# MGI-tech-bioinformatics/SuperPlus

Hardware: AMD Instinct MI355X
Metric: k-mers/s (DF createDict stage: trim + canonical k-mer count + solid filter + spectrum + adjacency) (higher is better)
Workload: dtype u64

## Files before the change

superplus_amd/csrc/dfk.hip:

```cpp
#include "../../include/dfk.h"
#include "dfk_kernels.h"
#include "dfk_arena.h"
#include "dfk_adj_plan.h"

#include <algorithm>
#include <chrono>
#include <cstdarg>
#include <cstdio>
#include <cstdlib>
#include <cstring>
#include <atomic>
#include <fcntl.h>
#include <functional>
#include <new>
#include <string>
#include <sys/mman.h>
#include <sys/stat.h>
#include <unistd.h>
#include <condition_variable>
#include <memory>
#include <mutex>
#include <numeric>
#include <thread>
#include <vector>
// ... 214 lines not shown
int device_scan(dfk_ctx* c, const uint64_t* in, uint64_t* out, uint64_t n)
{
    constexpr uint64_t PER = (uint64_t)SCAN_THREADS * SCAN_ITEMS;
    if (n == 0) return 0;
    const uint64_t nblk = (n + PER - 1) / PER;
    if (nblk == 1) {
        hipLaunchKernelGGL(k_scan_blocks, dim3(1), dim3(SCAN_THREADS), 0, c->stream, in, out, n, (uint64_t*)nullptr);
        HIP_TRY(hipGetLastError());
        return 0;
    }
    DevBuf sums; int rc = c->alloc(sums, nblk * 8, "scan block sums"); if (rc) return rc;
    hipLaunchKernelGGL(k_scan_blocks, dim3((unsigned)nblk), dim3(SCAN_THREADS), 0, c->stream, in, out, n, (uint64_t*)sums.p);
    HIP_TRY(hipGetLastError());
    rc = device_scan(c, (const uint64_t*)sums.p, (uint64_t*)sums.p, nblk); if (rc) return rc;
    hipLaunchKernelGGL(k_scan_add, dim3((unsigned)nblk), dim3(SCAN_THREADS), 0, c->stream, out, n, (const uint64_t*)sums.p);
    HIP_TRY(hipGetLastError());
    HIP_TRY(hipStreamSynchronize(c->stream));
    c->release(sums);
    return 0;
}

struct BucketTable {
    uint32_t log2_nb = 0;
    DevBuf acc;
    DevBuf summ;
    DevBuf classes;
    DevBuf ovf_list; uint64_t n_ovf = 0;
    DevBuf class_hist;
    std::vector<uint64_t> h_class;
    uint64_t n_records = 0, n_inst = 0;
};
struct Partition {
    DevBuf records, base, ipre, items;
    uint64_t n_records = 0, n_inst = 0, n_items = 0;
    uint64_t nb = 0;
};

template <int K>
PartParams part_params(const dfk_ctx* c, uint32_t log2_nb, uint32_t log2_world, int64_t read_id0, uint32_t sub_lo, uint32_t sub_n)
{
    const uint32_t M = c->cfg.minimizer_len;
    return PartParams{M, (uint32_t)K - M + 1, log2_nb, log2_world, read_id0, sub_lo, sub_n,
                      sweep_class_mask(sub_lo, sub_n, log2_nb - log2_world)};
}

int table_totals(dfk_ctx* c, const DevBuf& acc, uint64_t nb, uint64_t* n_records, uint64_t* n_inst)
{
    DevBuf tot; int rc = c->alloc(tot, 16, "bucket totals"); if (rc) return rc;
    HIP_TRY(hipMemsetAsync(tot.p, 0, 16, c->stream));
    hipLaunchKernelGGL(k_sum_acc, dim3(1024), dim3(256), 0, c->stream, (const unsigned long long*)acc.p, nb, (unsigned long long*)tot.p);
    HIP_TRY(hipGetLastError());
    uint64_t h[2];
    HIP_TRY(hipMemcpyAsync(h, tot.p, 16, hipMemcpyDeviceToHost, c->stream));
    HIP_TRY(hipStreamSynchronize(c->stream));
    c->release(tot);
    *n_records = h[0]; *n_inst = h[1];
    return 0;
}

struct ScanJob {
    PartParams pp; ScanPlan plan;
    DevBuf ovf_tmp, d_n;
    DevBuf keys, keys2, fill, sub;
    uint64_t n_pieces = 0; bool count_due = false;
    hipEvent_t ev_scan = nullptr, ev_count = nullptr, ev_part[2] = {nullptr, nullptr};
    std::vector<std::pair<hipEvent_t, hipEvent_t>> ev;
    ~ScanJob()
    {
        for (auto& e : ev) { (void)hipEventDestroy(e.first); (void)hipEventDestroy(e.second); }
        for (hipEvent_t e : {ev_scan, ev_count, ev_part[0], ev_part[1]}) if (e) (void)hipEventDestroy(e);
    }
};

template <int K> bool scan_takes_ranges(const dfk_ctx* c) { return c->cfg.minimizer_len == 16; }

ScanSwitches scan_switches()
{
    static const uint32_t scan_blocks = getenv("DFK_SCAN_BLOCKS") ? (uint32_t)atoi(getenv("DFK_SCAN_BLOCKS")) : 0;
    ScanSwitches sw;
    sw.scan_blocks = scan_blocks;
    if (const char* e = getenv("DFK_SCAN_KEY_PIECE")) { sw.key_piece_set = true; sw.key_piece = strtoull(e, nullptr, 10); }
    if (const char* e = getenv("DFK_SCAN_KEY_TAIL")) sw.key_tail = strtoull(e, nullptr, 10);
    sw.no_overlap = getenv("DFK_NO_OVERLAP") != nullptr;
    return sw;
}

template <int K>
int scan_begin(dfk_ctx* c, const Inputs& in, uint32_t log2_world, int64_t read_id0, BucketTable* T, bool by_class, ScanJob* J)
{
    J->pp = part_params<K>(c, T->log2_nb, log2_world, read_id0, 0, 1u << (T->log2_nb - log2_world));
    J->plan = plan_scan(ScanInputs{K, J->pp.W, T->log2_nb, log2_world, in.n_reads, in.packed_bytes, by_class, scan_takes_ranges<K>(c), c->stream2 != nullptr, scan_switches()});
    ScanPlan& P = J->plan;
    int rc = 0;
    if (by_class) { rc = c->alloc(T->class_hist, P.n_bins * 8, "class counters", Place::Low); if (rc) return rc; HIP_TRY(hipMemsetAsync(T->class_hist.p, 0, P.n_bins * 8, c->stream)); }
    else { rc = c->alloc(T->acc, P.nb * 8, "bucket counters", Place::Low); if (rc) return rc; }
    rc = c->alloc(T->summ, std::max<uint64_t>(1, in.n_reads) * 16, "run summaries", Place::Low); if (rc) return rc;
    rc = c->alloc(T->classes, std::max<uint64_t>(1, in.n_reads) * 4, "read bucket classes", Place::Low); if (rc) return rc;
    if (!by_class) HIP_TRY(hipMemsetAsync(T->acc.p, 0, P.nb * 8, c->stream));
    rc = c->alloc(J->ovf_tmp, P.ovf_cap * 4, "overflow read list (scratch)"); if (rc) return rc;
    rc = c->alloc(J->d_n, 16, "overflow read count"); if (rc) return rc;
    HIP_TRY(hipMemsetAsync(J->d_n.p, 0, 16, c->stream));
    if (P.keyed) {
        size_scan_keys(P, c->largest_allocatable());
        rc = c->alloc(J->keys, P.keys_bytes, "run keys (scratch)"); if (rc) return rc;
        rc = c->alloc(J->keys2, P.keys2_bytes, "run keys by sub-slice (scratch)"); if (rc) return rc;
        rc = c->alloc(J->fill, P.fill_bytes, "run key slice fills (scratch)"); if (rc) return rc;
        rc = c->alloc(J->sub, P.sub_bytes, "run key sub-slices (scratch)"); if (rc) return rc;
        if (P.n_slices > 1)
            for (hipEvent_t* e : {&J->ev_scan, &J->ev_count, &J->ev_part[0], &J->ev_part[1]}) HIP_TRY(hipEventCreateWithFlags(e, hipEventDisableTiming));
        TRACE("run keys: %u x %u classes of %llu keys, %u sub-slices each, pieces of %llu reads", P.n_slices, P.n_cls, (unsigned long long)P.cap,
              P.n_sub, (unsigned long long)P.piece_reads);
    }
    return 0;
}

inline int scan_keys_count(dfk_ctx* c, BucketTable* T, ScanJob* J)
{
    const ScanPlan& P = J->plan;
    const uint64_t n_subs = P.n_subs();
    const auto* off = (const unsigned long long*)J->sub.p + n_subs;
    if (P.n_slices > 1) HIP_TRY(hipStreamWaitEvent(c->stream, J->ev_part[scan_piece_step(P, J->n_pieces - 1).slice], 0));
    hipLaunchKernelGGL(k_keys_count, dim3((unsigned)n_subs), dim3(1024), 0, c->stream,
                       (const uint32_t*)J->keys2.p, off, P.sb, (unsigned long long*)T->acc.p);
    HIP_TRY(hipGetLastError());
    if (P.n_slices > 1) HIP_TRY(hipEventRecord(J->ev_count, c->stream));
    J->count_due = false;
    return 0;
}

template <int K>
int scan_keys_piece(dfk_ctx* c, const Inputs& in, BucketTable* T, ScanJob* J, uint64_t r0, uint64_t r1)
{
    const ScanPlan& P = J->plan;
    const unsigned cus = (unsigned)c->prop.multiProcessorCount;
    const unsigned grid = scan_grid(P, r1 - r0, cus);
    const uint64_t n_subs = P.n_subs();
    const bool two = P.n_slices > 1;
    const PieceStep step = scan_piece_step(P, J->n_pieces);
    const uint32_t sl = step.slice;
    hipStream_t ks = two ? c->stream2 : c->stream;
    auto* cnt = (unsigned long long*)J->sub.p;
    auto* off = cnt + n_subs;
    auto* cur = off + n_subs + 1;
    ScanKeys sk{(uint32_t*)J->keys.p + (uint64_t)sl * P.cap * P.n_cls, (unsigned long long*)J->fill.p + (uint64_t)sl * P.n_cls, P.cap, P.ib};
    if (step.wait_slice_reader) HIP_TRY(hipStreamWaitEvent(c->stream, J->ev_part[sl], 0));
    HIP_TRY(hipMemsetAsync(sk.fill, 0, P.n_cls * 8, c->stream));
    hipLaunchKernelGGL(HIP_KERNEL_NAME(k_scan_count<K, 16, true>), dim3(grid), dim3(PART_THREADS), scan_lds(P), c->stream,
                       in.packed, in.packed_bytes, in.base_off, (const uint32_t*)c->good_len.p, r0, r1, J->pp,
                       (unsigned long long*)T->acc.p, (unsigned long long*)nullptr, (unsigned long long*)J->d_n.p, P.ovf_cap,
                       (uint32_t*)J->ovf_tmp.p, (uint4*)T->summ.p, (uint32_t*)T->classes.p, sk);
    HIP_TRY(hipGetLastError());
    if (two) {
        HIP_TRY(hipEventRecord(J->ev_scan, c->stream));
        if (J->count_due) { int rc = scan_keys_count(c, T, J); if (rc) return rc; }
        HIP_TRY(hipStreamWaitEvent(ks, J->ev_scan, 0));
        if (step.wait_prev_count) HIP_TRY(hipStreamWaitEvent(ks, J->ev_count, 0));
    }
    HIP_TRY(hipMemsetAsync(cnt, 0, n_subs * 8, ks));
    const dim3 per_class(std::max(1u, 16u * cus / P.n_cls), P.n_cls);
    const uint32_t sh = 6 + P.sb;
    hipLaunchKernelGGL(k_keys_subcount, per_class, dim3(256), P.n_sub * 4, ks,
                       (const uint32_t*)sk.keys, (const unsigned long long*)sk.fill, sk.cap, sh, P.n_sub, cnt);
    HIP_TRY(hipGetLastError());
    hipLaunchKernelGGL(k_keys_offsets, dim3(1), dim3(1024), 0, ks, (const unsigned long long*)cnt, (uint32_t)n_subs, off, cur);
    HIP_TRY(hipGetLastError());
    hipLaunchKernelGGL(k_keys_partition, per_class, dim3(256), P.n_sub * 12, ks,
                       (const uint32_t*)sk.keys, (const unsigned long long*)sk.fill, sk.cap, sh, P.n_sub, cur, (uint32_t*)J->keys2.p);
    HIP_TRY(hipGetLastError());
    if (two) HIP_TRY(hipEventRecord(J->ev_part[sl], ks));
    ++J->n_pieces; J->count_due = true;
    if (!two) return scan_keys_count(c, T, J);
    return 0;
}

template <int K>
int scan_range(dfk_ctx* c, const Inputs& in, BucketTable* T, ScanJob* J, uint64_t r0, uint64_t r1)
{
    if (r1 <= r0) return 0;
    const PartParams& pp = J->pp;
    const ScanPlan& P = J->plan;
    const unsigned grid = scan_grid(P, r1 - r0, (unsigned)c->prop.multiProcessorCount);
    hipEvent_t e0, e1;
    HIP_TRY(hipEventCreate(&e0)); HIP_TRY(hipEventCreate(&e1));
    J->ev.emplace_back(e0, e1);
    HIP_TRY(hipEventRecord(e0, c->stream));
    if (P.keyed) {
        uint64_t p0 = r0;
        for (uint64_t m : scan_piece_sizes(P, r1 - r0, r1 == in.n_reads)) {
            int rc = scan_keys_piece<K>(c, in, T, J, p0, p0 + m); if (rc) return rc;
            p0 += m;
        }
        if (r1 == in.n_reads && J->count_due) { int rc = scan_keys_count(c, T, J); if (rc) return rc; }
    } else if (P.register_scan) {
        hipLaunchKernelGGL(HIP_KERNEL_NAME(k_scan_count<K, 16, false>), dim3(grid), dim3(PART_THREADS), scan_lds(P), c->stream,
                           in.packed, in.packed_bytes, in.base_off, (const uint32_t*)c->good_len.p, r0, r1, pp,
                           (unsigned long long*)T->acc.p, (unsigned long long*)T->class_hist.p, (unsigned long long*)J->d_n.p, P.ovf_cap,
                           (uint32_t*)J->ovf_tmp.p, (uint4*)T->summ.p, (uint32_t*)T->classes.p, ScanKeys{});
    } else {
        if (r0 != 0 || r1 != in.n_reads) return fail(DFK_E_STATE, "the general scan takes every read at once");
        hipLaunchKernelGGL(HIP_KERNEL_NAME(k_partition<K, false>), dim3(grid), dim3(PART_THREADS), scan_lds(P), c->stream,
                           in.packed, in.packed_bytes, in.base_off, (const uint32_t*)c->good_len.p, in.bc,
                           (int64_t)c->cfg.ign_bc_below, in.n_reads, pp, (unsigned long long*)T->acc.p, (unsigned long long*)T->class_hist.p,
                           (unsigned long long*)J->d_n.p, P.ovf_cap, (uint4*)J->ovf_tmp.p, (uint4*)T->summ.p,
                           (const uint32_t*)nullptr, (uint64_t)0, (const uint64_t*)nullptr, (uint32_t*)T->classes.p);
    }
    HIP_TRY(hipGetLastError());
    HIP_TRY(hipEventRecord(e1, c->stream));
    return 0;
}

template <int K>
int scan_end(dfk_ctx* c, const Inputs& in, uint64_t n_inst, BucketTable* T, ScanJob* J)
{
    int rc = 0;
    T->n_ovf = 0;
    if (J->count_due) { rc = scan_keys_count(c, T, J); if (rc) return rc; }
    c->release(J->keys); c->release(J->keys2); c->release(J->fill); c->release(J->sub);
    if (in.n_reads) {
        HIP_TRY(hipMemcpyAsync(&T->n_ovf, J->d_n.p, 8, hipMemcpyDeviceToHost, c->stream));
        HIP_TRY(hipStreamSynchronize(c->stream));
        if (T->n_ovf > J->plan.ovf_cap) {
            c->release(J->ovf_tmp);
            rc = c->alloc(J->ovf_tmp, in.n_reads * 4, "overflow read list (scratch)"); if (rc) return rc;
            HIP_TRY(hipMemsetAsync(J->d_n.p, 0, 16, c->stream));
            hipLaunchKernelGGL(k_select_overflow, dim3((unsigned)std::min<uint64_t>((in.n_reads + 255) / 256, 8192)), dim3(256), 0, c->stream,
                               (const uint4*)T->summ.p, in.n_reads, (uint32_t*)J->ovf_tmp.p, (unsigned long long*)J->d_n.p);
            HIP_TRY(hipGetLastError());
            HIP_TRY(hipMemcpyAsync(&T->n_ovf, J->d_n.p, 8, hipMemcpyDeviceToHost, c->stream));
            HIP_TRY(hipStreamSynchronize(c->stream));
        }
        if (T->n_ovf) {
            rc = c->alloc(T->ovf_list, T->n_ovf * 4, "overflow read list", Place::Low); if (rc) return rc;
            HIP_TRY(hipMemcpyAsync(T->ovf_list.p, J->ovf_tmp.p, T->n_ovf * 4, hipMemcpyDeviceToDevice, c->stream));
            HIP_TRY(hipStreamSynchronize(c->stream));
        }
    }
    c->release(J->ovf_tmp); c->release(J->d_n);
    HIP_TRY(hipStreamSynchronize(c->stream));
    float ms = 0;
    for (auto& e : J->ev) { float m = 0; if (hipEventElapsedTime(&m, e.first, e.second) == hipSuccess) ms += m; }
    c->st.ms_part_count = ms; c->st.reserved[6] = J->ev.size();
    TRACE("%llu of %llu reads have more than %d runs", (unsigned long long)T->n_ovf, (unsigned long long)in.n_reads, SUMMARY_RUNS);
    const uint64_t nb = J->plan.nb, n_bins = J->plan.n_bins;
    if (J->plan.by_class) {
        T->h_class.assign(n_bins, 0);
        HIP_TRY(hipMemcpyAsync(T->h_class.data(), T->class_hist.p, n_bins * 8, hipMemcpyDeviceToHost, c->stream));
        HIP_TRY(hipStreamSynchronize(c->stream));
        T->n_records = T->n_inst = 0;
        for (uint64_t i = 0; i < n_bins / 2; ++i) { T->n_records += T->h_class[i]; T->n_inst += T->h_class[n_bins / 2 + i]; }
    } else { rc = table_totals(c, T->acc, nb, &T->n_records, &T->n_inst); if (rc) return rc; }
    TRACE("partition count pass done (%llu buckets, %llu records%s)", (unsigned long long)nb, (unsigned long long)T->n_records, J->ev.size() > 1 ? ", in ranges under the upload" : "");
    if (T->n_inst != n_inst)
        return fail(DFK_E_HIP, "partition count pass saw %llu instances, trim saw %llu%s",
                    (unsigned long long)T->n_inst, (unsigned long long)n_inst,
                    (n_inst - T->n_inst) % (1ull << 32) == 0 ? " (a fine bucket with 2^32 or more instances: its counter keeps 32 bits)" : "");
    c->st.n_records = T->n_records; c->st.n_buckets = nb;
    return 0;
}

template <int K>
int partition_count(dfk_ctx* c, const Inputs& in, uint64_t n_inst, uint32_t log2_world, int64_t read_id0, BucketTable* T, bool by_class = false)
{
    ScanJob J;
    int rc = scan_begin<K>(c, in, log2_world, read_id0, T, by_class, &J); if (rc) return rc;
    rc = scan_range<K>(c, in, T, &J, 0, in.n_reads); if (rc) return rc;
    return scan_end<K>(c, in, n_inst, T, &J);
}

int pass_tables(dfk_ctx* c, const DevBuf& acc, uint32_t log2_sub, uint32_t world, uint32_t sub_lo, uint32_t sub_n, uint64_t budget, Partition* P)
{
    P->nb = (uint64_t)world * sub_n;
    const uint64_t nb = P->nb;
    DevBuf rec, inst, flags, idx;
    int rc = c->alloc(rec, (nb + 1) * 8, "bucket record counts"); if (rc) return rc;
    rc = c->alloc(inst, (nb + 1) * 8, "bucket instance counts"); if (rc) return rc;
    rc = c->alloc(P->base, (nb + 1) * 8, "bucket bases"); if (rc) return rc;
    rc = c->alloc(P->ipre, (nb + 1) * 8, "bucket instance prefix"); if (rc) return rc;
// ... 1564 lines not shown
```

superplus_amd/csrc/dfk_kernels.h:

```cpp
#pragma once
#include <type_traits>
#include "dfk_device.h"
#include "dfk_fallback.h"
#include "dfk_scan_plan.h"

namespace dfk {

template <int K>
__global__ void __launch_bounds__(256)
k_trim(const uint8_t* __restrict__ pq, const uint64_t* __restrict__ pq_off, uint64_t pq_nbytes,
       const uint64_t* __restrict__ base_off, uint64_t packed_bytes, const uint32_t* __restrict__ read_len,
       uint64_t n_reads, uint32_t min_qual, uint32_t* __restrict__ good_len,
       unsigned long long* __restrict__ n_inst, unsigned int* __restrict__ bad,
       unsigned long long* __restrict__ sum_good)
{
    unsigned long long mine = 0, good = 0;
    bool any_bad = false;
    for (uint64_t r = (uint64_t)blockIdx.x * blockDim.x + threadIdx.x; r < n_reads; r += (uint64_t)gridDim.x * blockDim.x) {
        uint32_t gl = 0;
        uint64_t p = pq_off[r], end = pq_off[r + 1];
        uint32_t idx = 0, run = 0;
        const uint64_t b0 = base_off[r], b1 = base_off[r + 1];
        bool ok = p <= end && end <= pq_nbytes && b0 <= b1 && b1 <= packed_bytes && b1 - b0 >= ((uint64_t)read_len[r] + 3) / 4;
        if (!ok) end = p;
// ... 11 lines not shown
                idx += nQs;
            } else {
                uint64_t bit = 8 * (p + 1) + 9;
                const uint32_t fmask = (1u << nBits) - 1u;
                for (uint32_t left = nQs; left;) {
                    const uint64_t by = bit >> 3;
                    const uint32_t sh = (uint32_t)(bit & 7);
                    uint64_t w = 0;
                    if (by + 8 <= pq_nbytes) __builtin_memcpy(&w, pq + by, 8);
                    else for (uint32_t k = 0; k < 8 && by + k < pq_nbytes; ++k) w |= (uint64_t)pq[by + k] << (8 * k);
                    w >>= sh;
                    const uint32_t n = min(left, (64u - sh) / nBits);
                    for (uint32_t i = 0; i < n; ++i, w >>= nBits) {
                        const uint32_t q = minQ + ((uint32_t)w & fmask);
                        if (q < min_qual) run = 0;
                        else if (++run >= (uint32_t)K) gl = idx + 1;
                        ++idx;
                    }
                    bit += (uint64_t)n * nBits; left -= n;
                }
            }
            p += blk;
        }
        uint32_t rl = read_len[r];
        if (!ok || idx != rl) { any_bad = true; gl = 0; }
        if (gl > rl) gl = rl;
        good_len[r] = gl;
        good += gl;
        if (gl >= (uint32_t)K + 1) mine += gl - K + 1;
    }
    __shared__ unsigned long long sh[2][4];
    __shared__ unsigned int sh_bad;
    if (threadIdx.x == 0) sh_bad = 0;
    __syncthreads();
#pragma unroll
    for (int d = 32; d > 0; d >>= 1) { mine += __shfl_down(mine, d, 64); good += __shfl_down(good, d, 64); }
    if ((threadIdx.x & 63) == 0) { sh[0][threadIdx.x >> 6] = mine; sh[1][threadIdx.x >> 6] = good; }
    if (any_bad) atomicOr(&sh_bad, 1u);
    __syncthreads();
    if (threadIdx.x == 0) {
        unsigned long long a0 = sh[0][0] + sh[0][1] + sh[0][2] + sh[0][3], a1 = sh[1][0] + sh[1][1] + sh[1][2] + sh[1][3];
        if (a0) atomicAdd(n_inst, a0);
        if (a1) atomicAdd(sum_good, a1);
        if (sh_bad) atomicOr(bad, 1u);
    }
}

struct PartParams {
    uint32_t M;
    uint32_t W;
    uint32_t log2_nb;
    uint32_t log2_world;
    int64_t  read_id0;
    uint32_t sub_lo;
    uint32_t sub_n;
    uint32_t class_mask;
};

constexpr uint32_t SWEEP_CLASSES = 32;
__host__ __device__ inline uint32_t sweep_class_of(uint32_t local_bucket, uint32_t log2_local)
{ return log2_local > 5 ? local_bucket >> (log2_local - 5) : local_bucket; }
__host__ __device__ inline uint32_t sweep_class_mask(uint32_t sub_lo, uint32_t sub_n, uint32_t log2_local)
{
    if (sub_n == 0) return 0u;
    const uint32_t a = sweep_class_of(sub_lo, log2_local), b = sweep_class_of(sub_lo + sub_n - 1, log2_local);
    const uint32_t upto_b = b >= 31 ? 0xFFFFFFFFu : ((1u << (b + 1)) - 1u);
    return upto_b & ~((1u << a) - 1u);
}

constexpr uint32_t SUMMARY_OVERFLOW = 15;

__device__ __forceinline__ uint32_t pass_local(uint32_t bucket, const PartParams& pp)
{
    const uint32_t ls = pp.log2_nb - pp.log2_world;
    const uint32_t d = (bucket & ((1u << ls) - 1u)) - pp.sub_lo;
    return d < pp.sub_n ? (bucket >> ls) * pp.sub_n + d : 0xFFFFFFFFu;
}

__device__ __forceinline__ uint32_t bucket_of(uint32_t minhash, const PartParams& pp)
{
    const uint32_t b = (minhash * 0x9E3779B1u) >> (32 - pp.log2_nb);
    return ((b & ((1u << pp.log2_world) - 1u)) << (pp.log2_nb - pp.log2_world)) | (b >> pp.log2_world);
}
constexpr int PART_QCAP = 8;

template <int K>
__device__ __forceinline__ void emit_record(const uint32_t* __restrict__ words, uint64_t n_words, uint64_t bit0,
                                            uint32_t s0, uint32_t nk, uint32_t bucket, uint32_t gl, int32_t tag,
                                            uint64_t dst_index, uint4* __restrict__ records)
{
    const bool hp = s0 > 0;
    const bool hs = s0 + nk + (uint32_t)K <= gl;
    uint64_t bo = bit0 + 2ull * (hp ? s0 - 1 : 0);
    uint64_t wi = bo >> 5; uint32_t sh = (uint32_t)bo & 31u;
    uint32_t w[7];
#pragma unroll
    for (int i = 0; i < 7; ++i) w[i] = (wi + i < n_words) ? words[wi + i] : 0u;
    uint32_t o[6];
#pragma unroll
    for (int i = 0; i < 6; ++i) o[i] = alignbit(w[i + 1], w[i], sh);
    if (!hp) {
#pragma unroll
        for (int i = 5; i > 0; --i) o[i] = (o[i] << 2) | (o[i - 1] >> 30);
        o[0] <<= 2;
    }
    uint32_t nbits = 2u * (1u + nk + (uint32_t)K - 1u + (hs ? 1u : 0u));
#pragma unroll
    for (int i = 0; i < 6; ++i) {
        uint32_t lo = 32u * i;
        if (nbits <= lo) o[i] = 0;
        else if (nbits < lo + 32u) o[i] &= (1u << (nbits - lo)) - 1u;
    }
    uint4 a{rec_header(nk, hp, hs, bucket), (uint32_t)tag, o[0], o[1]};
    uint4 b{o[2], o[3], o[4], o[5]};
    records[2 * dst_index] = a;
    records[2 * dst_index + 1] = b;
}

__device__ __forceinline__ uint32_t class_bin(uint32_t bucket, const PartParams& pp)
{
    const uint32_t ls = pp.log2_nb - pp.log2_world;
    const uint32_t sub = bucket & ((1u << ls) - 1u);
    return (bucket >> ls) * PART_CLASSES + (ls > 6 ? sub >> (ls - 6) : sub);
}

template <int K, bool WRITE>
__device__ __forceinline__ void
partition_read(uint64_t r, uint32_t* smem, uint32_t* __restrict__ lh,
            const uint8_t* __restrict__ packed, uint64_t packed_bytes, const uint64_t* __restrict__ base_off,
            const uint32_t* __restrict__ good_len, const int32_t* __restrict__ bc, int64_t ign_bc_below,
            uint64_t n_reads, const PartParams& pp,
            unsigned long long* __restrict__ bucket_acc, unsigned long long* __restrict__ bucket_cur, uint64_t n_out,
            uint4* __restrict__ records, uint4* __restrict__ summaries, const uint32_t* __restrict__ read_list, uint64_t n_list,
            const uint64_t* __restrict__ slice_base, uint32_t* __restrict__ read_classes)
{
    auto place = [&](uint32_t b) -> uint64_t {
        if (!slice_base) { const uint64_t d = atomicAdd(&bucket_cur[b], 1ull); return d < n_out ? d : ~0ull; }
        const uint32_t owner = b / pp.sub_n;
        const uint64_t d = slice_base[owner] + atomicAdd(&bucket_cur[owner], 1ull);
        return d < slice_base[owner + 1] ? d : ~0ull;
    };
    uint32_t* arr = smem;
    uint32_t* queue = smem + pp.W * PART_THREADS;
    uint8_t* sidx = reinterpret_cast<uint8_t*>(smem + pp.W * PART_THREADS);
    uint32_t* ring = reinterpret_cast<uint32_t*>(sidx + pp.W * PART_THREADS);
    uint64_t sum_lo = 0, sum_hi = 0;
    const int tid = threadIdx.x;
    if (WRITE && read_list) { if (r >= n_list) return; r = read_list[r]; }
    const uint32_t M = pp.M, W = pp.W;
    const uint32_t gl = r < n_reads ? good_len[r] : 0;
    if (gl < (uint32_t)K + 1) {
        if (!WRITE && r < n_reads) { summaries[r] = uint4{0, 0, 0, 0}; if (read_classes) read_classes[r] = 0u; }
        return;
    }
    uint32_t Pi = 0, cur_rel = 0;
    uint32_t cmask = 0;
    const uint32_t log2_local = pp.log2_nb - pp.log2_world;

    const uint64_t byte0 = base_off[r];
    const uint32_t* words = reinterpret_cast<const uint32_t*>(packed);
    const uint64_t n_words = (packed_bytes + 3) >> 2;
    const uint64_t bit0 = byte0 * 8;
    int32_t tag = -1;
    if (bc && (int64_t)r + pp.read_id0 >= ign_bc_below) tag = bc[r];

    const uint32_t mmask = M == 16 ? 0xFFFFFFFFu : ((1u << (2 * M)) - 1u);
// ... 82 lines not shown
        if (++bi == W) {
            uint32_t run = h, ri = W - 1;
            if (!WRITE) sidx[(W - 1) * PART_THREADS + tid] = (uint8_t)(W - 1);
            for (int i0 = (int)W - 2; i0 >= 0; i0 -= 8) {
                uint32_t v[8];
#pragma unroll
                for (int k = 0; k < 8; ++k) v[k] = i0 - k >= 0 ? arr[(i0 - k) * PART_THREADS + tid] : 0u;
#pragma unroll
                for (int k = 0; k < 8; ++k) {
                    const int i = i0 - k;
                    if (i >= 0) {
                        const bool lt = v[k] < run;
                        run = lt ? v[k] : run;
                        arr[i * PART_THREADS + tid] = run;
                        if (!WRITE) { ri = lt ? (uint32_t)i : ri; sidx[i * PART_THREADS + tid] = (uint8_t)ri; }
                    }
                }
            }
            bi = 0;
        }
        if (bi + 1 < W) sfx_next = arr[(bi + 1) * PART_THREADS + tid];
    }
    close_run();
    if (!WRITE) {
        const uint64_t lo = sum_lo | (qn <= (uint32_t)SUMMARY_RUNS ? qn : SUMMARY_OVERFLOW), hi = sum_hi;
        summaries[r] = uint4{(uint32_t)lo, (uint32_t)(lo >> 32), (uint32_t)hi, (uint32_t)(hi >> 32)};
        if (read_classes) read_classes[r] = cmask;
        if (qn > (uint32_t)SUMMARY_RUNS && bucket_cur) {
            const unsigned long long at = atomicAdd(bucket_cur, 1ull);
            if (at < n_out) reinterpret_cast<uint32_t*>(records)[at] = (uint32_t)r;
        }
    }
    if (WRITE) {
        for (uint32_t e = 0; e < qn; ++e) {
            uint32_t a = queue[(2 * e) * PART_THREADS + tid], b = queue[(2 * e + 1) * PART_THREADS + tid];
            const uint64_t dst = place(b);
            if (dst != ~0ull) emit_record<K>(words, n_words, bit0, a & 0xFFFFu, a >> 16, b, gl, tag, dst, records);
        }
    }
}

template <int K, bool WRITE>
__global__ void __launch_bounds__(PART_THREADS)
k_partition(const uint8_t* __restrict__ packed, uint64_t packed_bytes, const uint64_t* __restrict__ base_off,
            const uint32_t* __restrict__ good_len, const int32_t* __restrict__ bc, int64_t ign_bc_below,
            uint64_t n_reads, PartParams pp,
            unsigned long long* __restrict__ bucket_acc,
            unsigned long long* __restrict__ class_hist,
            unsigned long long* __restrict__ bucket_cur,
            uint64_t n_out,
            uint4* __restrict__ records,
            uint4* __restrict__ summaries,
            const uint32_t* __restrict__ read_list,
            uint64_t n_list,
            const uint64_t* __restrict__ slice_base,
            uint32_t* __restrict__ read_classes)
{
    extern __shared__ uint32_t smem[];
    uint32_t* lh = nullptr;
    const uint32_t n_bins = 2u * (PART_CLASSES << pp.log2_world);
    if (!WRITE && class_hist) {
        lh = reinterpret_cast<uint32_t*>(reinterpret_cast<uint8_t*>(smem) + 5 * pp.W * PART_THREADS + 4 * PART_RING * PART_THREADS);
        for (uint32_t i = threadIdx.x; i < n_bins; i += PART_THREADS) lh[i] = 0;
        __syncthreads();
    }
    const uint64_t n_work = (WRITE && read_list) ? n_list : n_reads;
    for (uint64_t r0 = (uint64_t)blockIdx.x * PART_THREADS; r0 < n_work; r0 += (uint64_t)gridDim.x * PART_THREADS)
        partition_read<K, WRITE>(r0 + threadIdx.x, smem, lh, packed, packed_bytes, base_off, good_len, bc, ign_bc_below, n_reads, pp,
                                 bucket_acc, bucket_cur, n_out, records, summaries, read_list, n_list, slice_base, read_classes);
    if (lh) {
        __syncthreads();
        for (uint32_t i = threadIdx.x; i < n_bins; i += PART_THREADS) if (lh[i]) atomicAdd(&class_hist[i], (unsigned long long)lh[i]);
    }
}

template <int I, int N, class F>
__device__ __forceinline__ void static_for(F&& f)
{
    if constexpr (I < N) { f(std::integral_constant<int, I>{}); static_for<I + 1, N>(f); }
}

constexpr uint32_t KEY_TILE = 4096;

template <int K, int M, bool KEYS>
__global__ void __launch_bounds__(PART_THREADS)
k_scan_count(const uint8_t* __restrict__ packed, uint64_t packed_bytes, const uint64_t* __restrict__ base_off,
             const uint32_t* __restrict__ good_len, uint64_t r_first, uint64_t n_reads , PartParams pp,
             unsigned long long* __restrict__ bucket_acc, unsigned long long* __restrict__ class_hist,
             unsigned long long* __restrict__ ovf_count, uint64_t ovf_cap, uint32_t* __restrict__ ovf_list,
             uint4* __restrict__ summaries, uint32_t* __restrict__ read_classes, ScanKeys sk)
{
    constexpr int W = K - M + 1;
    constexpr uint32_t mmask = M == 16 ? 0xFFFFFFFFu : ((1u << (2 * M)) - 1u);
    constexpr uint32_t rsh = 2 * (M - 1);
    constexpr int RUNS = SUMMARY_RUNS;
    static_assert(KTraits<K>::NK_MAX < 64, "nk takes the key's six low bits");
    extern __shared__ uint32_t smem[];
    uint32_t* runb = smem;
    uint16_t* runf = reinterpret_cast<uint16_t*>(runb + RUNS * PART_THREADS);
    uint32_t* const after_runs = reinterpret_cast<uint32_t*>(runf + RUNS * PART_THREADS);
    uint32_t* lh = nullptr;
    const uint32_t n_bins = 2u * (PART_CLASSES << pp.log2_world);
    if (class_hist) {
        lh = after_runs;
        for (uint32_t i = threadIdx.x; i < n_bins; i += PART_THREADS) lh[i] = 0;
        __syncthreads();
    }
    const int tid = threadIdx.x;
    uint32_t* st_key = after_runs;
    unsigned long long* st_base = reinterpret_cast<unsigned long long*>(st_key + SCAN_STAGE);
    uint32_t* st_h = reinterpret_cast<uint32_t*>(st_base + PART_CLASSES);
    uint32_t* st_n = st_h + PART_CLASSES;
    uint8_t* st_cls = reinterpret_cast<uint8_t*>(st_n + 1);
    const uint32_t n_cls = 1u << (pp.log2_nb - sk.ib);
    if constexpr (KEYS) {
        if (tid < PART_CLASSES) st_h[tid] = 0;
        if (tid == 0) *st_n = 0;
        __syncthreads();
    }
    auto flush = [&]() {
        const uint32_t n = *st_n;
        if (tid < (int)n_cls) { const uint32_t h = st_h[tid]; if (h) st_base[tid] = atomicAdd(&sk.fill[tid], (unsigned long long)h); st_h[tid] = 0; }
        __syncthreads();
        for (uint32_t j = tid; j < n; j += PART_THREADS) {
            const uint32_t key = st_key[j], cls = st_cls[j];
            const unsigned long long at = st_base[cls] + atomicAdd(&st_h[cls], 1u);
            if (at < sk.cap) sk.keys[cls * sk.cap + at] = key;
            else atomicAdd(&bucket_acc[(cls << sk.ib) | (key >> 6)], (1ull << 32) | (key & 63u));
        }
        __syncthreads();
        if (tid < (int)n_cls) st_h[tid] = 0;
        if (tid == 0) *st_n = 0;
        __syncthreads();
    };
    const uint32_t* words = reinterpret_cast<const uint32_t*>(packed);
    const uint64_t n_words = (packed_bytes + 3) >> 2;
    const uint32_t log2_local = pp.log2_nb - pp.log2_world;
    for (uint64_t r0 = r_first + (uint64_t)blockIdx.x * PART_THREADS; r0 < n_reads; r0 += (uint64_t)gridDim.x * PART_THREADS) {
        const uint64_t r = r0 + tid;
        const uint32_t gl = r < n_reads ? good_len[r] : 0;
        const bool live = gl >= (uint32_t)K + 1;
        uint32_t qn = 0, cmask = 0;
        uint64_t sum_lo = 0, sum_hi = 0;
        if (live) {
            const uint64_t bit0 = base_off[r] * 8;
            constexpr int NW = (2 * W + 30 + 31) / 32, NA = (2 * W + 31) / 32;
            auto load = [&](uint64_t bit, uint32_t (&w)[NW]) {
                const uint64_t wi = bit >> 5;
#pragma unroll
                for (int k = 0; k < NW; ++k) {
                    const uint64_t i = wi + k;
                    const uint32_t v = words[i < n_words ? i : n_words - 1];
                    w[k] = i < n_words ? v : 0u;
                }
            };
            uint64_t nbit = bit0 + 2 * (M - 1);
            uint32_t nw[NW];
            load(nbit, nw);
            uint32_t f = 0, rc = 0;
            {
                const uint64_t wi = bit0 >> 5;
                const uint32_t w0 = words[wi < n_words ? wi : n_words - 1], w1 = words[wi + 1 < n_words ? wi + 1 : n_words - 1];
                const uint32_t pw = alignbit(wi + 1 < n_words ? w1 : 0u, wi < n_words ? w0 : 0u, (uint32_t)bit0 & 31u);
#pragma unroll
                for (int j = 0; j < M - 1; ++j) { const uint32_t b = (pw >> (2 * j)) & 3u; f = ((f << 2) | b) & mmask; rc = (rc >> 2) | ((3u - b) << rsh); }
            }
            const uint32_t n_mmers = gl - M + 1;
            uint32_t arr[W], sidxw[(W + 3) / 4];
            auto sidx_get = [&](int i) -> uint32_t { return (sidxw[i >> 2] >> (8 * (i & 3))) & 255u; };
            auto sidx_set = [&](int i, uint32_t v) { const uint32_t sh = 8u * (uint32_t)(i & 3); sidxw[i >> 2] = (sidxw[i >> 2] & ~(255u << sh)) | (v << sh); };
#pragma unroll
            for (int i = 0; i < (W + 3) / 4; ++i) sidxw[i] = 0;
            uint32_t P = 0, Pi = 0;
            uint32_t cur_b = 0, cur_nk = 0, cur_rel = 0;
            auto close_run = [&]() {
                if (qn < (uint32_t)RUNS) {
                    runb[qn * PART_THREADS + tid] = cur_b;
                    runf[qn * PART_THREADS + tid] = (uint16_t)(cur_nk | (cur_rel << 6));
                } else {
                    if (lh) { const uint32_t bin = class_bin(cur_b, pp); atomicAdd(&lh[bin], 1u); atomicAdd(&lh[(PART_CLASSES << pp.log2_world) + bin], cur_nk); }
                    else atomicAdd(&bucket_acc[cur_b], (1ull << 32) | cur_nk);
                    cmask |= 1u << sweep_class_of(cur_b & ((1u << log2_local) - 1u), log2_local);
                }
                ++qn;
            };
            for (uint32_t t0 = 0; t0 < n_mmers; t0 += W) {
                uint32_t a[NA];
                {
                    const uint32_t sh = (uint32_t)nbit & 31u;
#pragma unroll
                    for (int i = 0; i < NA; ++i) a[i] = alignbit(i + 1 < NW ? nw[i + 1] : 0u, nw[i], sh);
                }
                nbit += 2 * W;
                load(nbit, nw);
                static_for<0, W>([&](auto bi_c) {
                    constexpr int bi = decltype(bi_c)::value;
                    if (t0 + (uint32_t)bi < n_mmers) {
                        const uint32_t b = (a[(2 * bi) >> 5] >> ((2 * bi) & 31)) & 3u;
                        f = ((f << 2) | b) & mmask;
                        rc = (rc >> 2) | ((3u - b) << rsh);
                        const uint32_t h = mmer_hash(f < rc ? f : rc);
                        const bool newmin = bi == 0 || h < P;
                        P = newmin ? h : P;
                        Pi = newmin ? (uint32_t)bi : Pi;
                        const bool first = t0 == 0;
                        if (!first || bi == W - 1) {
                            uint32_t mv = P;
                            bool older = false;
                            if constexpr (bi != W - 1) { older = arr[bi + 1] < mv; mv = older ? arr[bi + 1] : mv; }
                            const uint32_t bucket = bucket_of(mv, pp);
                            const bool open = first || bucket != cur_b || cur_nk == (uint32_t)KTraits<K>::NK_MAX;
                            if (open && !first) close_run();
                            const uint32_t rel = (bi != W - 1 && older) ? sidx_get(bi + 1 < W ? bi + 1 : 0) - (uint32_t)bi - 1u : (uint32_t)(W - 1 - bi) + Pi;
                            cur_rel = open ? rel : cur_rel;
                            cur_nk = open ? 1u : cur_nk + 1u;
                            cur_b = open ? bucket : cur_b;
                        }
                        arr[bi] = h;
                        if (bi == W - 1) {
                            uint32_t run = h, ri = W - 1;
                            sidx_set(W - 1, W - 1);
                            static_for<0, W - 1>([&](auto j_c) {
                                constexpr int i = W - 2 - decltype(j_c)::value;
                                const bool lt = arr[i] < run; run = lt ? arr[i] : run; arr[i] = run; ri = lt ? (uint32_t)i : ri; sidx_set(i, ri);
                            });
                        }
                    }
                });
            }
            close_run();
        }
        const uint32_t mine = min(qn, (uint32_t)RUNS);
        for (uint32_t i = 0; KEYS ? __syncthreads_or(i < mine) != 0 : __ballot(i < mine) != 0ull; ++i) {
            const bool has = i < mine;
            uint32_t cb = 0, nk = 0;
            if (has) {
                cb = runb[i * PART_THREADS + tid];
                const uint64_t fld = runf[i * PART_THREADS + tid];
                nk = (uint32_t)fld & 63u;
                const uint32_t bfld = 8u + 12u * i;
                if (bfld < 64u) { sum_lo |= fld << bfld; if (bfld > 52u) sum_hi |= fld >> (64u - bfld); } else sum_hi |= fld << (bfld - 64u);
                if constexpr (!KEYS) {
                    if (lh) { const uint32_t bin = class_bin(cb, pp); atomicAdd(&lh[bin], 1u); atomicAdd(&lh[(PART_CLASSES << pp.log2_world) + bin], nk); }
                    else atomicAdd(&bucket_acc[cb], (1ull << 32) | nk);
                }
                cmask |= 1u << sweep_class_of(cb & ((1u << log2_local) - 1u), log2_local);
            }
            if constexpr (KEYS) {
                const uint64_t m = __ballot(has);
                if (m) {
                    const uint32_t rk = __builtin_amdgcn_mbcnt_hi((uint32_t)(m >> 32), __builtin_amdgcn_mbcnt_lo((uint32_t)m, 0u));
                    const int lead = __ffsll((unsigned long long)m) - 1;
                    uint32_t at = 0;
                    if (has && rk == 0) at = atomicAdd(st_n, (uint32_t)__popcll(m));
                    at = __shfl(at, lead) + rk;
                    if (has) {
                        const uint32_t cls = cb >> sk.ib;
                        st_key[at] = ((cb & ((1u << sk.ib) - 1u)) << 6) | nk;
                        st_cls[at] = (uint8_t)cls;
                        atomicAdd(&st_h[cls], 1u);
                    }
                }
                __syncthreads();
                if (*st_n > (uint32_t)(SCAN_STAGE - PART_THREADS)) flush();
            }
        }
        if (r < n_reads) {
            const uint64_t lo = sum_lo | (qn <= (uint32_t)SUMMARY_RUNS ? qn : SUMMARY_OVERFLOW);
            summaries[r] = uint4{(uint32_t)lo, (uint32_t)(lo >> 32), (uint32_t)sum_hi, (uint32_t)(sum_hi >> 32)};
            if (read_classes) read_classes[r] = cmask;
        }
        if (qn > (uint32_t)SUMMARY_RUNS) {
            const unsigned long long at = atomicAdd(ovf_count, 1ull);
            if (at < ovf_cap) ovf_list[at] = (uint32_t)r;
        }
    }
    if constexpr (KEYS) { __syncthreads(); if (*st_n) flush(); }
    if (lh) {
        __syncthreads();
        for (uint32_t i = threadIdx.x; i < n_bins; i += PART_THREADS) if (lh[i]) atomicAdd(&class_hist[i], (unsigned long long)lh[i]);
    }
}

constexpr int KEY_VECS = 4;
static_assert(KEY_TILE == 256u * 4u * KEY_VECS, "a tile is KEY_VECS 16-byte vectors per thread of a 256-thread block");
__device__ __forceinline__ uint32_t key_vec_n(uint64_t t0, uint64_t t1, int j)
{
    const uint64_t i = t0 + ((uint64_t)j * 256u + threadIdx.x) * 4u;
    return i < t1 ? (uint32_t)min((uint64_t)4, t1 - i) : 0u;
}
__device__ __forceinline__ void key_tile_load(const uint32_t* __restrict__ k, uint64_t t0, uint64_t t1, uint4 (&v)[KEY_VECS])
{
#pragma unroll
    for (int j = 0; j < KEY_VECS; ++j) {
        const uint64_t i = t0 + ((uint64_t)j * 256u + threadIdx.x) * 4u;
        v[j] = i < t1 ? *reinterpret_cast<const uint4*>(k + i) : make_uint4(0u, 0u, 0u, 0u);
    }
}
template <typename F>
__device__ __forceinline__ void key_tile_each(uint64_t t0, uint64_t t1, const uint4 (&v)[KEY_VECS], F&& f)
{
#pragma unroll
    for (int j = 0; j < KEY_VECS; ++j) {
        const uint32_t m = key_vec_n(t0, t1, j);
        if (m > 0) f(v[j].x);
        if (m > 1) f(v[j].y);
        if (m > 2) f(v[j].z);
        if (m > 3) f(v[j].w);
        __builtin_amdgcn_sched_barrier(0);
    }
}

__global__ void __launch_bounds__(256)
k_keys_subcount(const uint32_t* __restrict__ keys, const unsigned long long* __restrict__ fill, uint64_t cap, uint32_t sh ,
// ... 1704 lines not shown
```

superplus_amd/csrc/dfk_scan_plan.h:

```cpp
#pragma once
#include <algorithm>
#include <cstddef>
#include <cstdint>
#include <vector>
#include "dfk_fallback.h"

namespace dfk {

constexpr int PART_THREADS = 128;
constexpr int PART_RING = 2;
constexpr int SUMMARY_RUNS = 10;
constexpr uint32_t PART_CLASSES = 64;

struct ScanKeys {
    uint32_t* keys;
    unsigned long long* fill;
    uint64_t cap;
    uint32_t ib;
};
constexpr int SCAN_STAGE = 1536;
constexpr uint32_t KEY_SUB_BITS = 14;
constexpr size_t SCAN_RUN_LDS = (sizeof(uint32_t) + sizeof(uint16_t)) * SUMMARY_RUNS * PART_THREADS;
constexpr size_t SCAN_STAGE_LDS = (sizeof(uint32_t) + 1) * SCAN_STAGE + (sizeof(unsigned long long) + sizeof(uint32_t)) * PART_CLASSES + sizeof(uint32_t);
static_assert(SCAN_RUN_LDS + SCAN_STAGE_LDS <= 16384, "ten scan blocks a CU (160 KB of LDS)");

constexpr uint64_t SCAN_TAIL_READS = 32ull << 20;
constexpr uint64_t KEY_SCRATCH_MAX = 16ull << 30;
constexpr uint32_t SCAN_BLOCKS_PER_CU = 128;

struct ScanSwitches {
    bool key_piece_set = false; uint64_t key_piece = 0;
    uint64_t key_tail = SCAN_TAIL_READS;
    uint32_t scan_blocks = 0;
    bool no_overlap = false;
};

struct ScanInputs {
    int K; uint32_t W, log2_nb, log2_world;
    uint64_t n_reads, packed_bytes;
    bool by_class;
    bool register_scan;
    bool second_stream;
    ScanSwitches sw;
};

struct ScanPlan {
    ScanSwitches sw;
    uint32_t W = 0; uint64_t nb = 0, n_bins = 0, ovf_cap = 0; bool by_class = false, register_scan = false;
    bool keyed = false; uint32_t n_cls = 0, ib = 0, sb = 0, n_sub = 0, n_slices = 1;
    double keys_per_read = 0.0;
    uint64_t n_reads = 0, cap = 0, piece_reads = 0, tail_reads = 0;
    uint64_t keys_bytes = 0, keys2_bytes = 0, fill_bytes = 0, sub_bytes = 0;
    uint64_t n_subs() const { return (uint64_t)n_cls * n_sub; }
};

inline uint64_t ovf_cap(uint64_t n_reads) { return n_reads / 16 + 1024; }

inline ScanPlan plan_scan(const ScanInputs& in)
{
    ScanPlan p;
    p.sw = in.sw; p.W = in.W; p.n_reads = in.n_reads; p.by_class = in.by_class; p.register_scan = in.register_scan;
    p.nb = 1ull << in.log2_nb;
    p.n_bins = 2ull * (PART_CLASSES << in.log2_world);
    p.ovf_cap = ovf_cap(in.n_reads);
    const double runs = in.n_reads ? 1.0 + 2.0 * std::max(0.0, 4.0 * (double)in.packed_bytes / (double)in.n_reads - in.K + 1) / (in.W + 1) : 0.0;
    p.keyed = !in.by_class && in.register_scan && in.n_reads && (runs >= 3.5 || in.sw.key_piece_set);
    if (!p.keyed) return p;
    const uint32_t cb = std::min<uint32_t>(6, in.log2_nb);
    p.ib = in.log2_nb - cb; p.n_cls = 1u << cb;
    p.sb = std::min(KEY_SUB_BITS, p.ib); p.n_sub = 1u << (p.ib - p.sb);
    p.keys_per_read = 1.25 * runs;
    p.n_slices = in.second_stream && !in.sw.no_overlap ? 2 : 1;
    p.tail_reads = in.sw.key_tail;
    return p;
}

inline void size_scan_keys(ScanPlan& p, uint64_t largest_allocatable)
{
    const double per_read = p.keys_per_read;
    const uint32_t copies = p.n_slices + 1;
    const uint64_t want = 4ull * copies * (uint64_t)(per_read * (double)p.n_reads) + 4ull * copies * p.n_cls;
    const uint64_t room = std::min<uint64_t>(std::min(want, KEY_SCRATCH_MAX), largest_allocatable / 3);
    p.cap = std::max<uint64_t>(1024, room / (4 * copies) / p.n_cls) & ~3ull;
    p.piece_reads = std::max<uint64_t>(PART_THREADS, (uint64_t)((double)(p.cap * p.n_cls) / per_read));
    if (p.sw.key_piece_set) p.piece_reads = std::max<uint64_t>(1, std::min<uint64_t>(p.piece_reads, p.sw.key_piece));
    p.keys_bytes = p.n_slices * p.cap * p.n_cls * 4;
    p.keys2_bytes = p.cap * p.n_cls * 4;
    p.fill_bytes = p.n_slices * p.n_cls * 8;
    p.sub_bytes = (3 * p.n_subs() + 1) * 8;
}

inline std::vector<uint64_t> scan_piece_sizes(const ScanPlan& p, uint64_t n, bool last)
{
    std::vector<uint64_t> tail;
    uint64_t t_sum = 0;
    if (last && p.n_slices > 1 && p.tail_reads)
        for (uint64_t t = p.tail_reads; t < p.piece_reads && t_sum + t < n; t *= 2) { tail.push_back(t); t_sum += t; }
    std::vector<uint64_t> v;
    const uint64_t body = n - t_sum, nb = (body + p.piece_reads - 1) / p.piece_reads;
    for (uint64_t i = 0, at = 0; i < nb; ++i) { const uint64_t e = body * (i + 1) / nb; v.push_back(e - at); at = e; }
    v.insert(v.end(), tail.rbegin(), tail.rend());
    return v;
}

struct PieceStep { uint32_t slice; bool wait_slice_reader, wait_prev_count; };

inline PieceStep scan_piece_step(const ScanPlan& p, uint64_t i)
{
    const bool two = p.n_slices > 1;
    return PieceStep{two ? (uint32_t)(i & 1) : 0u, two && i >= 2, two && i >= 1};
}

inline unsigned scan_grid(const ScanPlan& p, uint64_t n, unsigned cus)
{
    const uint64_t blocks = (n + PART_THREADS - 1) / PART_THREADS;
    const uint64_t per_cu = p.sw.scan_blocks ? p.sw.scan_blocks : p.keyed || p.by_class ? SCAN_BLOCKS_PER_CU : 0;
    return (unsigned)(per_cu ? std::min<uint64_t>(blocks, per_cu * cus) : blocks);
}

inline size_t scan_lds(const ScanPlan& p)
{
    if (p.keyed) return SCAN_RUN_LDS + SCAN_STAGE_LDS;
    const size_t window = (sizeof(uint32_t) + 1) * p.W * PART_THREADS + sizeof(uint32_t) * PART_RING * PART_THREADS;
    return (p.register_scan ? SCAN_RUN_LDS : window) + (p.by_class ? p.n_bins * 4 : 0);
}

inline uint32_t pick_log2_nb(uint64_t n_inst, uint32_t log2_world, uint64_t inst_per_bucket)
{
    uint32_t l = ceil_log2(n_inst / inst_per_bucket + 1);
    l = std::max<uint32_t>(l, 4 + log2_world);
    return std::min<uint32_t>(l, 28);
}

inline uint64_t upload_segment_bytes(uint64_t packed_bytes, uint64_t seg_switch)
{
    return seg_switch ? std::max<uint64_t>(64, seg_switch & ~63ull) : std::max<uint64_t>(256ull << 20, ((packed_bytes / 12) + (64ull << 20)) & ~((64ull << 20) - 1));
}

struct OffsetSampling { uint64_t stride, n_samp; };
inline OffsetSampling offset_sampling(uint64_t n_reads)
{
    const uint64_t stride = std::max<uint64_t>(1, (n_reads + 32767) / 32768);
    return OffsetSampling{stride, n_reads / stride + 2};
}

inline uint64_t reads_within(const std::vector<uint64_t>& samp, uint64_t stride, uint64_t n, uint64_t bytes)
{
    const uint64_t i = (uint64_t)(std::upper_bound(samp.begin(), samp.end(), bytes) - samp.begin());
    return i ? std::min<uint64_t>((i - 1) * stride, n) : 0;
// ... 4 lines not shown
```

Before: 65.72 billion.

## Streamline scan kernel m-mer rolling, single-rank bucket hashing, and run slot indexing

```diff
diff --git a/superplus_amd/csrc/dfk.hip b/superplus_amd/csrc/dfk.hip
--- a/superplus_amd/csrc/dfk.hip
+++ b/superplus_amd/csrc/dfk.hip
@@ -320,6 +320,7 @@
     if (const char* e = getenv("DFK_SCAN_KEY_PIECE")) { sw.key_piece_set = true; sw.key_piece = strtoull(e, nullptr, 10); }
     if (const char* e = getenv("DFK_SCAN_KEY_TAIL")) sw.key_tail = strtoull(e, nullptr, 10);
     sw.no_overlap = getenv("DFK_NO_OVERLAP") != nullptr;
+    sw.no_keys = getenv("DFK_SCAN_NO_KEYS") != nullptr;
     return sw;
 }
 
@@ -383,7 +384,8 @@
     ScanKeys sk{(uint32_t*)J->keys.p + (uint64_t)sl * P.cap * P.n_cls, (unsigned long long*)J->fill.p + (uint64_t)sl * P.n_cls, P.cap, P.ib};
     if (step.wait_slice_reader) HIP_TRY(hipStreamWaitEvent(c->stream, J->ev_part[sl], 0));
     HIP_TRY(hipMemsetAsync(sk.fill, 0, P.n_cls * 8, c->stream));
-    hipLaunchKernelGGL(HIP_KERNEL_NAME(k_scan_count<K, 16, true>), dim3(grid), dim3(PART_THREADS), scan_lds(P), c->stream,
+    if (J->pp.log2_world != 0) return fail(DFK_E_STATE, "run keys are built on one rank only");
+    hipLaunchKernelGGL(HIP_KERNEL_NAME(k_scan_count<K, 16, true, true>), dim3(grid), dim3(PART_THREADS), scan_lds(P), c->stream,
                        in.packed, in.packed_bytes, in.base_off, (const uint32_t*)c->good_len.p, r0, r1, J->pp,
                        (unsigned long long*)T->acc.p, (unsigned long long*)nullptr, (unsigned long long*)J->d_n.p, P.ovf_cap,
                        (uint32_t*)J->ovf_tmp.p, (uint4*)T->summ.p, (uint32_t*)T->classes.p, sk);
@@ -430,7 +432,8 @@
         }
         if (r1 == in.n_reads && J->count_due) { int rc = scan_keys_count(c, T, J); if (rc) return rc; }
     } else if (P.register_scan) {
-        hipLaunchKernelGGL(HIP_KERNEL_NAME(k_scan_count<K, 16, false>), dim3(grid), dim3(PART_THREADS), scan_lds(P), c->stream,
+        auto* scan = pp.log2_world == 0 ? k_scan_count<K, 16, false, true> : k_scan_count<K, 16, false, false>;
+        hipLaunchKernelGGL(scan, dim3(grid), dim3(PART_THREADS), scan_lds(P), c->stream,
                            in.packed, in.packed_bytes, in.base_off, (const uint32_t*)c->good_len.p, r0, r1, pp,
                            (unsigned long long*)T->acc.p, (unsigned long long*)T->class_hist.p, (unsigned long long*)J->d_n.p, P.ovf_cap,
                            (uint32_t*)J->ovf_tmp.p, (uint4*)T->summ.p, (uint32_t*)T->classes.p, ScanKeys{});
diff --git a/superplus_amd/csrc/dfk_kernels.h b/superplus_amd/csrc/dfk_kernels.h
--- a/superplus_amd/csrc/dfk_kernels.h
+++ b/superplus_amd/csrc/dfk_kernels.h
@@ -117,6 +117,12 @@
     const uint32_t b = (minhash * 0x9E3779B1u) >> (32 - pp.log2_nb);
     return ((b & ((1u << pp.log2_world) - 1u)) << (pp.log2_nb - pp.log2_world)) | (b >> pp.log2_world);
 }
+template <bool ONE_RANK>
+__device__ __forceinline__ uint32_t bucket_of(uint32_t minhash, const PartParams& pp)
+{
+    if constexpr (ONE_RANK) return (minhash * 0x9E3779B1u) >> (32 - pp.log2_nb);
+    else return bucket_of(minhash, pp);
+}
 constexpr int PART_QCAP = 8;
 
 template <int K>
@@ -365,8 +371,8 @@
 
 constexpr uint32_t KEY_TILE = 4096;
 
-template <int K, int M, bool KEYS>
-__global__ void __launch_bounds__(PART_THREADS)
+template <int K, int M, bool KEYS, bool ONE_RANK>
+__global__ void __launch_bounds__(PART_THREADS, K <= 40 ? 5 : 4)
 k_scan_count(const uint8_t* __restrict__ packed, uint64_t packed_bytes, const uint64_t* __restrict__ base_off,
              const uint32_t* __restrict__ good_len, uint64_t r_first, uint64_t n_reads , PartParams pp,
              unsigned long long* __restrict__ bucket_acc, unsigned long long* __restrict__ class_hist,
@@ -374,10 +380,10 @@
              uint4* __restrict__ summaries, uint32_t* __restrict__ read_classes, ScanKeys sk)
 {
     constexpr int W = K - M + 1;
-    constexpr uint32_t mmask = M == 16 ? 0xFFFFFFFFu : ((1u << (2 * M)) - 1u);
-    constexpr uint32_t rsh = 2 * (M - 1);
     constexpr int RUNS = SUMMARY_RUNS;
     static_assert(KTraits<K>::NK_MAX < 64, "nk takes the key's six low bits");
+    static_assert(M == 16, "an m-mer is one 32-bit window of the read's 2-bit stream");
+    static_assert(2 * PART_THREADS == 256, "a lane's slot cursor is 2 * tid + 256 * (runs closed)");
     extern __shared__ uint32_t smem[];
     uint32_t* runb = smem;
     uint16_t* runf = reinterpret_cast<uint16_t*>(runb + RUNS * PART_THREADS);
@@ -423,7 +429,7 @@
         const uint64_t r = r0 + tid;
         const uint32_t gl = r < n_reads ? good_len[r] : 0;
         const bool live = gl >= (uint32_t)K + 1;
-        uint32_t qn = 0, cmask = 0;
+        uint32_t qslot = 2u * (uint32_t)tid, cmask = 0;
         uint64_t sum_lo = 0, sum_hi = 0;
         if (live) {
             const uint64_t bit0 = base_off[r] * 8;
@@ -440,13 +446,14 @@
             uint64_t nbit = bit0 + 2 * (M - 1);
             uint32_t nw[NW];
             load(nbit, nw);
-            uint32_t f = 0, rc = 0;
+            uint32_t f = 0, before;
             {
                 const uint64_t wi = bit0 >> 5;
                 const uint32_t w0 = words[wi < n_words ? wi : n_words - 1], w1 = words[wi + 1 < n_words ? wi + 1 : n_words - 1];
                 const uint32_t pw = alignbit(wi + 1 < n_words ? w1 : 0u, wi < n_words ? w0 : 0u, (uint32_t)bit0 & 31u);
 #pragma unroll
-                for (int j = 0; j < M - 1; ++j) { const uint32_t b = (pw >> (2 * j)) & 3u; f = ((f << 2) | b) & mmask; rc = (rc >> 2) | ((3u - b) << rsh); }
+                for (int j = 0; j < M - 1; ++j) f = (f << 2) | ((pw >> (2 * j)) & 3u);
+                before = pw << 2;
             }
             const uint32_t n_mmers = gl - M + 1;
             uint32_t arr[W], sidxw[(W + 3) / 4];
@@ -454,18 +461,19 @@
             auto sidx_set = [&](int i, uint32_t v) { const uint32_t sh = 8u * (uint32_t)(i & 3); sidxw[i >> 2] = (sidxw[i >> 2] & ~(255u << sh)) | (v << sh); };
 #pragma unroll
             for (int i = 0; i < (W + 3) / 4; ++i) sidxw[i] = 0;
-            uint32_t P = 0, Pi = 0;
+            constexpr int PB = (2 * W - 1 <= 65 || !KEYS) ? W : 0;
+            uint32_t P = 0, PiW = 0;
             uint32_t cur_b = 0, cur_nk = 0, cur_rel = 0;
             auto close_run = [&]() {
-                if (qn < (uint32_t)RUNS) {
-                    runb[qn * PART_THREADS + tid] = cur_b;
-                    runf[qn * PART_THREADS + tid] = (uint16_t)(cur_nk | (cur_rel << 6));
+                if (qslot < 2u * RUNS * PART_THREADS) {
+                    *reinterpret_cast<uint32_t*>(reinterpret_cast<uint8_t*>(runb) + 2u * qslot) = cur_b;
+                    *reinterpret_cast<uint16_t*>(reinterpret_cast<uint8_t*>(runf) + qslot) = (uint16_t)(cur_nk | (cur_rel << 6));
                 } else {
                     if (lh) { const uint32_t bin = class_bin(cur_b, pp); atomicAdd(&lh[bin], 1u); atomicAdd(&lh[(PART_CLASSES << pp.log2_world) + bin], cur_nk); }
                     else atomicAdd(&bucket_acc[cur_b], (1ull << 32) | cur_nk);
                     cmask |= 1u << sweep_class_of(cur_b & ((1u << log2_local) - 1u), log2_local);
                 }
-                ++qn;
+                qslot += 2u * PART_THREADS;
             };
             for (uint32_t t0 = 0; t0 < n_mmers; t0 += W) {
                 uint32_t a[NA];
@@ -479,22 +487,27 @@
                 static_for<0, W>([&](auto bi_c) {
                     constexpr int bi = decltype(bi_c)::value;
                     if (t0 + (uint32_t)bi < n_mmers) {
-                        const uint32_t b = (a[(2 * bi) >> 5] >> ((2 * bi) & 31)) & 3u;
-                        f = ((f << 2) | b) & mmask;
-                        rc = (rc >> 2) | ((3u - b) << rsh);
+                        constexpr int wq = (2 * bi + 2) >> 5, ws = (2 * bi + 2) & 31;
+                        const uint32_t wlo = wq == 0 ? before : a[wq > 0 ? wq - 1 : 0];
+                        const uint32_t win = ws == 0 ? wlo : alignbit(a[wq < NA ? wq : NA - 1], wlo, ws);
+                        f = alignbit(f, win, 30);
+                        const uint32_t rc = ~win;
                         const uint32_t h = mmer_hash(f < rc ? f : rc);
+                        if constexpr (bi == W - 1) before = win;
                         const bool newmin = bi == 0 || h < P;
                         P = newmin ? h : P;
-                        Pi = newmin ? (uint32_t)bi : Pi;
+                        PiW = newmin ? (uint32_t)(bi + PB) : PiW;
                         const bool first = t0 == 0;
                         if (!first || bi == W - 1) {
                             uint32_t mv = P;
                             bool older = false;
                             if constexpr (bi != W - 1) { older = arr[bi + 1] < mv; mv = older ? arr[bi + 1] : mv; }
-                            const uint32_t bucket = bucket_of(mv, pp);
+                            const uint32_t bucket = bucket_of<ONE_RANK>(mv, pp);
                             const bool open = first || bucket != cur_b || cur_nk == (uint32_t)KTraits<K>::NK_MAX;
                             if (open && !first) close_run();
-                            const uint32_t rel = (bi != W - 1 && older) ? sidx_get(bi + 1 < W ? bi + 1 : 0) - (uint32_t)bi - 1u : (uint32_t)(W - 1 - bi) + Pi;
+                            uint32_t rel;
+                            if constexpr (PB == W) rel = ((bi != W - 1 && older) ? sidx_get(bi + 1 < W ? bi + 1 : 0) : PiW) - (uint32_t)(bi + 1);
+                            else rel = (bi != W - 1 && older) ? sidx_get(bi + 1 < W ? bi + 1 : 0) - (uint32_t)bi - 1u : (uint32_t)(W - 1 - bi) + PiW;
                             cur_rel = open ? rel : cur_rel;
                             cur_nk = open ? 1u : cur_nk + 1u;
                             cur_b = open ? bucket : cur_b;
@@ -513,6 +526,7 @@
             }
             close_run();
         }
+        const uint32_t qn = qslot >> 8;
         const uint32_t mine = min(qn, (uint32_t)RUNS);
         for (uint32_t i = 0; KEYS ? __syncthreads_or(i < mine) != 0 : __ballot(i < mine) != 0ull; ++i) {
             const bool has = i < mine;
diff --git a/superplus_amd/csrc/dfk_scan_plan.h b/superplus_amd/csrc/dfk_scan_plan.h
--- a/superplus_amd/csrc/dfk_scan_plan.h
+++ b/superplus_amd/csrc/dfk_scan_plan.h
@@ -33,6 +33,7 @@
     uint64_t key_tail = SCAN_TAIL_READS;
     uint32_t scan_blocks = 0;
     bool no_overlap = false;
+    bool no_keys = false;
 };
 
 struct ScanInputs {
@@ -64,7 +65,7 @@
     p.n_bins = 2ull * (PART_CLASSES << in.log2_world);
     p.ovf_cap = ovf_cap(in.n_reads);
     const double runs = in.n_reads ? 1.0 + 2.0 * std::max(0.0, 4.0 * (double)in.packed_bytes / (double)in.n_reads - in.K + 1) / (in.W + 1) : 0.0;
-    p.keyed = !in.by_class && in.register_scan && in.n_reads && (runs >= 3.5 || in.sw.key_piece_set);
+    p.keyed = !in.by_class && in.register_scan && in.n_reads && (runs >= 3.5 || in.sw.key_piece_set) && !in.sw.no_keys;
     if (!p.keyed) return p;
     const uint32_t cb = std::min<uint32_t>(6, in.log2_nb);
     p.ib = in.log2_nb - cb; p.n_cls = 1u << cb;
```

After: 67.02 billion (median of 6 runs). +2.0%, better.
